# 0xC0000054/pdn-jpegxl

Hardware: AMD Instinct MI355X
Metric: megapixels/sec decode (4K lossy VarDCT) (higher is better)
Workload: dtype f32

## Files before the change

### pdn_jpegxl_amd/api.py

```python
import ctypes as C
import os

import numpy as np

from . import build as _build

DECODER_STATUS = ["Ok", "NullParameter", "InvalidParameter", "OutOfMemory", "HasAnimation", "HasMultipleFrames",
                  "ImageDimensionExceedsInt32", "UnsupportedChannelFormat", "CreateLayerError", "CreateMetadataError",
                  "DecodeError", "MetadataError", "InvalidFileSignature"]
ENCODER_STATUS = ["Ok", "NullParameter", "OutOfMemory", "UserCanceled", "EncodeError", "WriteError"]
IMAGE_FORMAT = ["Gray", "Rgb", "Cmyk"]
KNOWN_PROFILE = ["Srgb", "LinearSrgb", "LinearGray", "GraySrgbTRC", "DisplayP3", "Rec709", "Rec2020Linear", "Rec2020PQ"]
S_OK, E_ABORT, E_OUTOFMEMORY, E_FAIL = 0, -2147467260, -2147024882, -2147467259


class ErrorInfo(C.Structure):
    _fields_ = [("errorMessage", C.c_char * 256)]


class BitmapData(C.Structure):
    _fields_ = [("scan0", C.c_void_p), ("width", C.c_uint32), ("height", C.c_uint32), ("stride", C.c_uint32)]


class EncoderOptions(C.Structure):
# ... 248 lines not shown
    L = lib()
    L.jxlhip_parse_metadata.restype = C.c_size_t
    L.jxlhip_parse_metadata.argtypes = [C.c_char_p, C.c_size_t, C.c_int32, C.c_void_p, C.c_size_t, C.POINTER(C.c_int32), C.POINTER(ErrorInfo)]
    err = ErrorInfo()
    st = C.c_int32(0)
    n = L.jxlhip_parse_metadata(data, len(data), which, None, 0, C.byref(st), C.byref(err))
    if st.value != 0 or n == 0:
        return DECODER_STATUS[st.value], None, err.errorMessage.decode("ascii", "replace")
    buf = (C.c_uint8 * n)()
    L.jxlhip_parse_metadata(data, len(data), which, buf, n, C.byref(st), C.byref(err))
    return DECODER_STATUS[st.value], bytes(buf), ""


def static_table(name, index, dtype):
    L = lib()
    n = L.jxlhip_static_table(name.encode(), index, None, 0)
    buf = np.empty(n // np.dtype(dtype).itemsize, dtype)
    L.jxlhip_static_table(name.encode(), index, buf.ctypes.data, n)
    return buf


_PLANE_DTYPES = {"lf": np.float32, "lf_quant": np.int32, "cellinfo": np.uint32, "raw_quant": np.uint16, "sharpness": np.uint8,
                 "ytox": np.int8, "ytob": np.int8, "alpha": np.uint8, "inv_sigma": np.float32, "qcoef": np.int32,
                 "xyb_idct": np.float32, "xyb_filtered": np.float32}


def _last_stage_times(fn_name):
    L = lib()
    fn = getattr(L, fn_name)
    fn.restype = C.c_int32
    fn.argtypes = [C.POINTER(C.c_char_p), C.POINTER(C.c_float), C.c_int32]
    names = (C.c_char_p * 32)()
    ms = (C.c_float * 32)()
    k = fn(names, ms, 32)
    return {names[i].decode(): ms[i] for i in range(k)}


def last_load_stage_times():
    return _last_stage_times("jxlhip_last_load_stage_times")


def last_save_stage_times():
    return _last_stage_times("jxlhip_last_save_stage_times")


class Decoder:

# ... 61 lines not shown
```

### pdn_jpegxl_amd/csrc/decoder.cc

```cpp
#include <hip/hip_runtime.h>
#include <algorithm>
#include <atomic>
#include <cmath>
#include <cstdarg>
#include <cstdio>
#include <cstdlib>
#include <cstring>
#include <memory>
#include <mutex>
#include <string>
#include <thread>
#include <vector>
#include "../../include/jxlfiletypeio.h"
#include "host_parse.h"
#include "icc.h"
#include "kernels.h"

namespace jxlhip {

struct HipError : std::runtime_error {
  explicit HipError(const std::string& m) : std::runtime_error(m) {}
};
#define HIP_OK(expr)                                                                                      \
  do {                                                                                                    \
// ... 430 lines not shown
  Bump blob, ws_zero, ws;
  int n_extra = 0;
  std::vector<int> first_extra((size_t)n, 0);
  for (int i = 0; i < n; i++) {
    first_extra[i] = n + n_extra;
    if (parse_status[i] == DecoderStatus_Ok && frames[i].encoding == 0) n_extra += (int)frames[i].extra_passes.size();
  }
  const size_t off_imgs = blob.Take(sizeof(DevImage) * (size_t)(n + n_extra));
  struct PassLayout {
    size_t a_cmap, a_cfg, a_alias, a_pfx[3] = {}, lz_hf = 0, scan[kNumQuantTables] = {}, centries, cblk, bitpos, hf_order;
  };
  struct PerImg {
    std::vector<PassLayout> extra;
    size_t m_direct = 0;
    size_t sec_off, sec_size, tree, m_cmap, m_cfg, m_alias, a_cmap, a_cfg, a_alias, order[kNumOrders][3], cs;
    size_t m_pfx[3] = {}, a_pfx[3] = {};
    size_t lz_lf = 0, lz_grp = 0, lz_hf = 0, lz_mod = 0;
    size_t scan[kNumQuantTables] = {};
    size_t trc_lut = 0;
    size_t dq[kNumQuantTables] = {};
    size_t z_cellinfo, z_status, centries, cblk, hf_order;
    std::vector<size_t> mod_planes;
    size_t mod_chan, mod_desc, wp_lf, wp_grp, lf_end, alpha32;
    size_t lf[3], lf_tmp[3], lfq[3], lf_extra, rawq, sharp, ytox, ytob, binfo, lf_desc, lf_count, alpha_desc, blk_list, blk_count, bitpos, tile_list, tmp[3], xyb[3], inv_sigma, alpha;
    size_t orient_tmp = 0;
    size_t layer_px = 0;
  };
  std::vector<PerImg> L((size_t)n);
  std::vector<size_t> file_cs((size_t)S.nfiles, 0);
  std::vector<uint8_t> cs_put((size_t)S.nfiles, 0);
  auto take_cs = [&](int i) {
    const ParsedFrame& f = frames[i];
    if (!f.is_layer) return blob.Take(f.cs_size + 16);
    size_t& o = file_cs[S.file_of[i]];
    if (!o) o = blob.Take(f.cs_size + 16) + 1;
    return o - 1;
  };
  const size_t z_status_base = ws_zero.Take((size_t)std::max(1, n) * 64);
  int total_lf = 0, total_groups = 0, n_mod_tasks = 0;
  int mod_lanes = 64, mod_rb = 0, mod_wp_lds = 0;
  size_t total_mod_sections = 0;
  for (int i = 0; i < n; i++) {
    if (parse_status[i] != DecoderStatus_Ok || frames[i].encoding != 1) continue;
    if (!frames[i].tree_row_static && frames[i].group_dim <= 256) mod_rb = 256;
    if (frames[i].tree_uses_wp && frames[i].group_dim <= 256) { mod_wp_lds = 1; mod_lanes = 8; }
    total_mod_sections += frames[i].single ? 1 : 1 + (size_t)frames[i].nlf + frames[i].ng;
  }
// ... 77 lines not shown
          if (l.dq[q] || !ep.custom_order[o][0].empty() || !ep.custom_order[o][1].empty() || !ep.custom_order[o][2].empty()) pl.scan[q] = blob.Take(8 * 3 * (size_t)dq_n[q], 256) + 1;
        }
        pl.centries = ws.Take((size_t)std::max(1, g1 - g0) * f.xg * kGroupEntriesCap * 4);
        pl.cblk = ws.Take(3 * cells * sizeof(U32x2));
        pl.bitpos = ws.Take((size_t)f.ng * 8);
        pl.hf_order = blob.Take(4 * (size_t)std::max<uint32_t>(1, f.ng));
        l.extra.push_back(pl);
      }
    }
    for (int c = 0; c < 3; c++) { l.lf[c] = ws.Take(4 * cells); l.lf_tmp[c] = ws.Take(4 * cells); l.lfq[c] = ws.Take(4 * cells); }
    l.lf_extra = ws.Take(f.nlf);
    l.rawq = ws.Take(2 * cells);
    l.sharp = ws.Take(cells);
    l.ytox = ws.Take(tiles);
    l.ytob = ws.Take(tiles);
    l.binfo = ws.Take((size_t)f.nlf * kBinfoInts * 4);
    l.lf_desc = ws.Take((size_t)f.nlf * 8 * sizeof(ChanDesc));
    l.lf_count = ws.Take((size_t)f.nlf * 4);
    l.alpha_desc = ws.Take((size_t)f.ng * sizeof(ChanDesc));
    l.blk_list = ws.Take((size_t)f.ng * 1024 * 4);
    l.blk_count = ws.Take((size_t)f.ng * 4);
    l.bitpos = ws.Take((size_t)f.ng * 8);
    l.tile_list = ws.Take(tiles * 4);
    l.alpha32 = ws.Take(4 * (size_t)f.xsize * f.ysize);
    chunk_pix = std::max(chunk_pix, pix);
    l.inv_sigma = ws.Take(4 * cells);
    l.alpha = ws.Take((size_t)f.xsize * f.ysize * OutBytesPerSample(f));
    if (f.is_layer) l.layer_px = ws.Take((size_t)f.xsize * f.ysize * (f.ncolor + (f.alpha_index >= 0 ? 1 : 0)) * OutBytesPerSample(f));
    l.lf_end = ws.Take(8);
    if (f.tree_uses_wp) { l.wp_lf = ws.Take((size_t)f.nlf * kWpLfInts * 4); l.wp_grp = ws.Take((size_t)f.ng * 10 * (kGroupDim + 2) * 4); }
    {
      int b0 = 0, b1 = (int)f.yg;
      if (band_rows > 0) { b0 = std::min<int>(band_first_row, (int)f.yg); b1 = std::min<int>(b0 + band_rows, (int)f.yg); }
      const int g0 = std::max(0, b0 - 1), g1 = std::min<int>((int)f.yg, b1 + 1);
      total_lf += ((g1 + 7) / 8 - g0 / 8) * (int)f.xlf;
      total_groups += (g1 - g0) * (int)f.xg * (int)f.num_passes;
    }
  }
  const int pixel_chunk = debug_taps ? std::max(1, n) : std::min(std::max(1, n), kPixelChunk);
  std::vector<size_t> chunk_tmp((size_t)pixel_chunk * 3), chunk_xyb((size_t)pixel_chunk * 3), chunk_coef((size_t)pixel_chunk * 3);
  if (chunk_pix)
    for (int k = 0; k < pixel_chunk * 3; k++) { chunk_tmp[k] = ws.Take(4 * chunk_pix); chunk_xyb[k] = ws.Take(4 * chunk_pix); chunk_coef[k] = ws.Take(4 * chunk_pix); }
  for (int i = 0; i < n; i++)
    if (parse_status[i] == DecoderStatus_Ok && band_rows > 0 && (band_first_row < 0 || band_first_row >= (int)frames[i].yg)) {
      parse_status[i] = DecoderStatus_DecodeError;
      parse_msg[i] = "band decode: the first group row lies outside the frame";
// ... 335 lines not shown
        double a = 0;
        for (int j = 0; j < 3; j++) a += (double)plan.from_srgb[r * 3 + j] * (double)f.opsin_inv[j * 3 + k];
        d.opsin_inv[r * 3 + k] = (float)a * (255.0f / f.intensity_target);
      }
    for (int k = 0; k < 3; k++) { d.opsin_bias[k] = f.opsin_bias[k]; d.opsin_bias_cbrt[k] = std::cbrt(f.opsin_bias[k]); }
    d.cellinfo = (uint32_t*)(wz + l.z_cellinfo);
    d.status = (uint32_t*)(wz + l.z_status);
    status_off[i] = l.z_status;
    for (int c = 0; c < 3; c++) {
      d.coef[c] = (int32_t*)(wr + chunk_coef[(size_t)(i % pixel_chunk) * 3 + c]);
      d.lf[c] = (float*)(wr + l.lf[c]); d.lf_tmp[c] = (float*)(wr + l.lf_tmp[c]); d.lfq[c] = (int32_t*)(wr + l.lfq[c]);
      d.lf_final[c] = d.skip_lf_smoothing ? d.lf[c] : d.lf_tmp[c];
      d.tmp[c] = (float*)(wr + chunk_tmp[(size_t)(i % pixel_chunk) * 3 + c]); d.xyb[c] = (float*)(wr + chunk_xyb[(size_t)(i % pixel_chunk) * 3 + c]);
      d.xyb2[c] = (float*)d.coef[c];
    }
    d.lf_extra = wr + l.lf_extra;
    d.rawq = (uint16_t*)(wr + l.rawq); d.sharp = wr + l.sharp;
    d.ytox = (int8_t*)(wr + l.ytox); d.ytob = (int8_t*)(wr + l.ytob);
    d.binfo = (int32_t*)(wr + l.binfo);
    d.lf_desc = (ChanDesc*)(wr + l.lf_desc); d.lf_count = (uint32_t*)(wr + l.lf_count); d.alpha_desc = (ChanDesc*)(wr + l.alpha_desc);
    d.blk_list = (uint32_t*)(wr + l.blk_list); d.blk_count = (uint32_t*)(wr + l.blk_count);
    d.grp_bitpos = (uint64_t*)(wr + l.bitpos);
    d.tile_list = (uint32_t*)(wr + l.tile_list);
    d.alpha32 = (int32_t*)(wr + l.alpha32);
    d.centries = (uint32_t*)(wr + l.centries); d.centries_g0 = d.dec_gy0 * (int32_t)f.xg;
    d.cblk = (U32x2*)(wr + l.cblk);
    d.inv_sigma = (float*)(wr + l.inv_sigma);
    d.alpha = wr + l.alpha;
    d.lf_end_bits = (uint64_t*)(wr + l.lf_end);
    d.alpha_in_global = (d.has_alpha && f.ng == 1) ? 1 : 0;
    d.lf_start_bits = f.after_lf_global_bits;
    if (f.single) {
      d.single = 1;
      d.hf_start_bits = f.hf_start_bits;
    }
    if (f.tree_uses_wp) { d.wp_lf = (int32_t*)(wr + l.wp_lf); d.wp_grp = (int32_t*)(wr + l.wp_grp); d.wp_grp_ints = 10 * (kGroupDim + 2); }
    d.out = f.orientation == 1 ? dev_out[i] : wr + l.orient_tmp;
    if (f.is_layer) d.out = wr + l.layer_px;
    float** cur = d.xyb;
    float** other = d.xyb2;
    d.fused_gab_epf1 = (!debug_taps && f.epf_iters >= 1) ? (f.epf_iters == 1 ? 1 : 2) : 0;
    d.stream_no_gab = (d.fused_gab_epf1 && (!f.gab || f.epf_iters == 3)) ? 1 : 0;
    d.stage_on[0] = (f.gab && (!d.fused_gab_epf1 || f.epf_iters == 3)) ? 1 : 0;
    d.stage_on[1] = f.epf_iters == 3;
    d.stage_on[2] = f.epf_iters >= 1 && !d.fused_gab_epf1;
    d.stage_on[3] = f.epf_iters >= 2 && !d.fused_gab_epf1;
// ... 184 lines not shown
      if (s_lf != s_hf) HIP_OK(hipStreamWaitEvent(xs, S.lf_done, 0));
      LaunchInterference(kind, wgs, lds_kb, ms, xbuf, xbytes, xs);
    }
  }
#endif
  Mark("hf_start", s_hf, 1);
  if (!(skip_stages & 2))
  LaunchHfDecode(d_imgs, (const SectionTask*)(d_blob + off_pass_tasks), npass_t, hf_waves * 64, lane_stride, hf_ring, lds_hf <= kLdsMax ? lds_hf : 0, lds_hf_lanes, s_hf);
  Mark("hf_decode", s_hf, 1);
  if (any_alpha && !(skip_stages & 4))
    LaunchAlphaAns(d_imgs, (const SectionTask*)(d_blob + off_alpha_tasks), nalpha_t, alpha_stride, lds_alpha <= kLdsMax ? lds_alpha : 0, direct_alpha, lean_mod, s_hf);
  Mark("alpha_ans", s_hf, 1);
  if (debug_taps) {
    taps.assign(n, Tap());
    LaunchExpandCoefficients(d_imgs, n, true, max_tiles, stream);
    HIP_OK(hipStreamSynchronize(stream));
    CopyPlaneTap(0);
  }
  const bool finish_on_hf = s_hf == stream || debug_taps || !Knob("JXLHIP_ALPHA_FINISH_ON_PIX");
  if (finish_on_hf) {
    if (any_alpha && !(skip_stages & 4)) LaunchAlphaFinish(d_imgs, n, max_groups, s_hf);
    Mark("alpha_finish", s_hf, 1);
  }
  if (s_hf != stream) {
    HIP_OK(hipEventRecord(S.hf_done, s_hf));
    HIP_OK(hipStreamWaitEvent(stream, S.hf_done, 0));
  }
  Mark("main_start", stream, 2);
  if (!finish_on_hf) {
    if (any_alpha && !(skip_stages & 4)) LaunchAlphaFinish(d_imgs, n, max_groups, stream);
    Mark("alpha_finish", stream, 2);
  }
  hipStream_t s_pix = (Knob("JXLHIP_PIX_ON_HF") && s_hf != stream) ? s_hf : stream;
  for (int c0 = 0; c0 < n; c0 += pixel_chunk) {
    const int cnt = std::min(pixel_chunk, n - c0);
    if (!(skip_stages & 8))
    LaunchReconTiles(d_imgs + c0, cnt, max_tiles, d_basis_all, d_basis_small, d_llf_scale, d_basis_mfma, s_pix);
    Mark("reconstruct", s_pix, 2);
    LaunchExpandCoefficients(d_imgs + c0, cnt, false, max_tiles, s_pix);
    LaunchGenericReconstruct(d_imgs + c0, cnt, d_basis_all, d_basis_small, d_llf_scale, s_pix);
    Mark("reconstruct_generic", s_pix, 2);
    if (debug_taps) { HIP_OK(hipStreamSynchronize(s_pix)); CopyPlaneTap(1); }
    if (!(skip_stages & 16))
    LaunchFilterTiles(d_imgs + c0, cnt, max_w, max_h, stage_mask, any_unfiltered, any_fused, any_fused2, s_pix);
    Mark("filters+output", s_pix, 2);
  }
// ... 289 lines not shown
}

size_t jxlhip_read_plane(JxlHipDecoder* dec, int32_t index, const char* name, int32_t channel, void* dst, size_t capacity) {
  if (!dec || !name) return 0;
  JxlHipDecoder::Slot& S = dec->Last();
  if (index < 0 || index >= S.n || S.pending) return 0;
  if (S.parse_status[index] != DecoderStatus_Ok) return 0;
  const DevImage& d = S.imgs[index];
  std::string nm(name);
  const size_t cells = (size_t)d.w8 * d.h8, pix = (size_t)d.wp * d.hp;
  const void* src = nullptr;
  size_t bytes = 0;
  bool host = false;
  const int c = std::min(2, std::max(0, channel));
  if (nm == "lf") { src = d.lf_final[c]; bytes = cells * 4; }
  else if (nm == "lf_quant") { src = d.lfq[c]; bytes = cells * 4; }
  else if (nm == "cellinfo") { src = d.cellinfo; bytes = cells * 4; }
  else if (nm == "raw_quant") { src = d.rawq; bytes = cells * 2; }
  else if (nm == "sharpness") { src = d.sharp; bytes = cells; }
  else if (nm == "ytox") { src = d.ytox; bytes = (size_t)d.wt * d.ht; }
  else if (nm == "ytob") { src = d.ytob; bytes = (size_t)d.wt * d.ht; }
  else if (nm == "alpha") { src = d.alpha; bytes = (size_t)d.w * d.h; }
  else if (nm == "inv_sigma") { src = d.inv_sigma; bytes = cells * 4; }
  else if (dec->debug_taps && (size_t)index < S.taps.size()) {
    host = true;
    if (nm == "qcoef") { src = S.taps[index].qcoef[c].data(); bytes = S.taps[index].qcoef[c].size(); }
    else if (nm == "xyb_idct") { src = S.taps[index].xyb_idct[c].data(); bytes = S.taps[index].xyb_idct[c].size(); }
    else if (nm == "xyb_filtered") { src = S.taps[index].xyb_filtered[c].data(); bytes = S.taps[index].xyb_filtered[c].size(); }
  }
  (void)pix;
  if (!src || !bytes) return 0;
  if (dst && capacity) {
    size_t nb = std::min(bytes, capacity);
    if (host) memcpy(dst, src, nb);
    else if (hipMemcpy(dst, src, nb, hipMemcpyDeviceToHost) != hipSuccess) return 0;
  }
  return bytes;
}

int32_t jxlhip_stage_times(JxlHipDecoder* dec, const char** names, float* ms, int32_t capacity) {
  if (!dec) return 0;
  JxlHipDecoder::Slot& S = dec->Last();
  int32_t k = 0;
  for (size_t i = 1; i < S.stage_names.size() && i < S.stage_ms.size() && k < capacity; i++) {
    if (S.stage_ms[i] < 0.f) continue;
    if (names) names[k] = S.stage_names[i].c_str();
// ... 211 lines not shown
```

### pdn_jpegxl_amd/csrc/dev_types.h

```cpp
#pragma once
#include <stdint.h>

namespace jxlhip {

constexpr int kNumStrategies = 27;
constexpr int kNumOrders = 13;
constexpr int kNumQuantTables = 17;
constexpr int kGroupDim = 256;
constexpr int kGroupBlocks = 32;
constexpr int kLfGroupBlocks = 256;
constexpr int kMaxClustersLds = 128;
constexpr uint32_t kGroupEntriesCap = 3u * 65536u;

enum DevError : uint32_t {
  kErrNone = 0,
  kErrBitstream = 1u << 0,
  kErrUnsupportedHeader = 1u << 1,
  kErrUnsupportedTree = 1u << 2,
  kErrBlockLayout = 1u << 3,
  kErrRange = 1u << 4,
  kErrUnsupportedTransform = 1u << 5,
};

struct alignas(8) U32x2 { uint32_t x, y; };

struct DevTreeNode {
  int32_t property;
  int32_t splitval;
  uint32_t a;
  uint32_t b;
};

struct DevCode {
  const uint8_t* ctx_map;
  const uint32_t* cfg;
// ... 110 lines not shown
  uint32_t* lz_lf;
  uint32_t* lz_grp;
  uint32_t* lz_hf;
  uint32_t* lz_mod;
  int32_t* alpha32;
  uint32_t* centries;
  int32_t centries_g0, pad2;
  U32x2* cblk;
  int32_t* coef[3];
  float* tmp[3];
  float* xyb[3];
  float* xyb2[3];
  float* inv_sigma;
  float* stage_in[5][3];
  float* stage_out[5][3];
  int32_t stage_on[5];
  int32_t final_stage;
  int32_t fused_gab_epf1;
  float* stream_in[3];
  float* stream_mid[3];
  int32_t stream_no_gab;
  int32_t stream_pairs;
  uint32_t* tile_list;
  uint8_t* alpha;
  uint8_t* out;
  uint32_t* status;
};

struct ComposeFrame {
  const float* px;
  int32_t x0, y0, w, h;
  int32_t mode[2];
  int32_t source[2];
  int32_t clamp[2];
  int32_t save;
  int32_t pad;
};
struct ComposeImage {
  int32_t w, h, nch, has_alpha;
  int32_t premul, orientation, out_bits, out_float;
  int32_t first, count;
  int32_t raw, pad0;
  uint8_t* out;
};

constexpr int kUniGridCells = 2048;
// ... 13 lines not shown
```

### pdn_jpegxl_amd/csrc/kernels.h

```cpp
#pragma once
#include <hip/hip_runtime.h>
#include "dev_types.h"

namespace jxlhip {

void LaunchLfAns(const DevImage* imgs, const SectionTask* tasks, int ntasks, int slots, size_t lds_bytes, int scalar_rows, bool lean, hipStream_t s);
void LaunchLfFinish(const DevImage* imgs, const SectionTask* tasks, int ntasks, hipStream_t s);
void LaunchHfBlockList(const DevImage* imgs, int nimg, int max_groups, hipStream_t s);
size_t HfLaneLdsBytes(int ring_words);
void LaunchHfDecode(const DevImage* imgs, const SectionTask* tasks, int nwg, int threads, int lane_stride, int ring_words, size_t lds_bytes,
                    size_t lane_bytes, hipStream_t s);
void LaunchAlphaAns(const DevImage* imgs, const SectionTask* tasks, int nwg, int lane_stride, size_t lds_bytes, int scalar_rows, bool lean, hipStream_t s);
void LaunchAlphaFinish(const DevImage* imgs, int nimg, int max_groups, hipStream_t s);
void LaunchModularAns(const DevImage* imgs, int nimg, const SectionTask* tasks, int ntasks, size_t lds_bytes, int max_sections, int max_coded,
                      int lanes, int rb_width, int wp_lds, int scalar_rows, hipStream_t s);
void LaunchModularOp(int kind, int32_t* a, int32_t* b, int32_t* c, int aw, int ah, int rw, int rh, int type, hipStream_t s);
void LaunchModularPalette(const int32_t* palette, const int32_t* index, int32_t* const* out, int nout, int nb_colors, int w, int h, uint32_t* status,
                          hipStream_t s);
void LaunchModularOut(const DevImage* imgs, int nimg, size_t max_pixels, hipStream_t s);
void LaunchOrient(const uint8_t* src, uint8_t* dst, int w, int h, int px_bytes, int orientation, hipStream_t s);
void LaunchLfPixelStages(const DevImage* imgs, int nimg, size_t max_cells, hipStream_t s);
void LaunchExpandCoefficients(const DevImage* imgs, int nimg, bool all_tiles, int max_tiles, hipStream_t s);
void LaunchGenericReconstruct(const DevImage* imgs, int nimg, const float* basis_all, const float* basis_small,
                              const float* llf_scale, hipStream_t s);
void LaunchReconTiles(const DevImage* imgs, int nimg, int max_tiles, const float* basis_all, const float* basis_small,
                      const float* llf_scale, const float* basis_mfma, hipStream_t s);
void LaunchFilterTiles(const DevImage* imgs, int nimg, int max_w, int max_h, int stage_mask, bool any_unfiltered,
                       int any_fused, int any_fused2, hipStream_t s);

void LaunchCompose(const ComposeImage* imgs, const ComposeFrame* frames, int nimg, int max_segments, hipStream_t s);

void LaunchStatusToHost(const uint32_t* src, uint32_t* dst_pinned, int nwords, hipStream_t s);
#ifdef JXLHIP_EXPERIMENTS
void LaunchInterference(int kind, int wg_per_cu, int lds_kb, float ms, float* scratch, size_t scratch_bytes, hipStream_t s);
#endif

}
```

### pdn_jpegxl_amd/csrc/tile_kernels.hip

```cpp
#include <hip/hip_runtime.h>
#include <cstdlib>
#include "dev_types.h"
#include "dev_util.h"
#include "kernels.h"

namespace jxlhip {

#ifndef JXLHIP_PRIO_PIXEL
#define JXLHIP_PRIO_PIXEL 0
#endif
#if JXLHIP_PRIO_PIXEL
#define JXL_PIXEL_PRIO() __builtin_amdgcn_s_setprio(JXLHIP_PRIO_PIXEL)
#else
#define JXL_PIXEL_PRIO() ((void)0)
#endif

namespace {

constexpr int kTS = 64;
constexpr int kLP = 65;

__device__ const uint8_t t_quant_table[kNumStrategies] = {0, 1, 2, 3, 4, 5, 6, 6, 7, 7, 8, 8, 9, 9, 10, 10, 10, 10, 11, 12, 12, 13, 14, 14, 15, 16, 16};

__device__ __forceinline__ bool Special(uint32_t s) { return (s >= 1 && s <= 3) || (s >= 12 && s <= 17); }
// ... 135 lines not shown
}

#define JXL_IDCT_STEP(Bp, v0, v1)                                                                  \
  {                                                                                                \
    const float4 b0 = *(const float4*)(Bp);                                                        \
    const float4 b1 = *(const float4*)((Bp) + 4);                                                  \
    a0[0] += v0 * b0.x; a0[1] += v0 * b0.y; a0[2] += v0 * b0.z; a0[3] += v0 * b0.w;                \
    a0[4] += v0 * b1.x; a0[5] += v0 * b1.y; a0[6] += v0 * b1.z; a0[7] += v0 * b1.w;                \
    a1[0] += v1 * b0.x; a1[1] += v1 * b0.y; a1[2] += v1 * b0.z; a1[3] += v1 * b0.w;                \
    a1[4] += v1 * b1.x; a1[5] += v1 * b1.y; a1[6] += v1 * b1.z; a1[7] += v1 * b1.w;                \
  }

__device__ __forceinline__ float DequantBias(int32_t v, float qb, float qb3) {
  if (v == 0) return 0.f;
  if (v == 1) return qb;
  if (v == -1) return -qb;
  const float f = (float)v;
  return f - qb3 * __builtin_amdgcn_rcpf(f);
}
typedef int __attribute__((ext_vector_type(4))) I4v;

constexpr int kTileF = kTS * kLP;

__global__ __launch_bounds__(768, 6) void recon_tile_kernel(const DevImage* __restrict__ imgs, const float* basis_all, const float* basis_small,
                                                             const float* llf_scale, const float* basis_mfma) {
  JXL_PIXEL_PRIO();
  extern __shared__ __align__(16) uint8_t smem_raw[];
  float* cfc3 = (float*)smem_raw;
  float* B816 = cfc3 + 3 * kTileF;
  float* cscale = B816 + 320;
  uint32_t* ci = (uint32_t*)(cscale + 64);
  uint32_t* cmeta = ci + 64;
  uint32_t* cnq = cmeta + 64;
  uint32_t* cpre = cnq + 64;
  uint32_t* cstart = cpre + 3 * 64;
  uint32_t* ctot = cstart + 3 * 64;
  const U32x2** csc = (const U32x2**)(ctot + 4);
  float4* t32_lo = (float4*)(csc + 64);
  float4* t32_hi = t32_lo + 128;
  float4* t64 = t32_hi + 128;
  const DevImage& im = imgs[blockIdx.y];
  const int tile = blockIdx.x;
  if (tile >= im.wt * im.ht) return;
  const int tid = threadIdx.x;
  const int tx = tile % im.wt, ty = tile / im.wt;
  if (ty < im.dec_gy0 * 4 || ty >= im.dec_gy1 * 4) return;
  const int wave = tid >> 6, lane = tid & 63, team = wave >> 2, tw = wave & 3;
  const int c = team == 0 ? 1 : (team == 1 ? 0 : 2);
  const int wp = im.wp, hp = im.hp;
  {
    float4* z = (float4*)cfc3;
    for (int i = tid; i < 3 * kTileF / 4; i += 768) z[i] = make_float4(0.f, 0.f, 0.f, 0.f);
  }
  int bad = 0, has64 = 0;
  if (tid < 64) {
    const int cx = tx * 8 + (tid & 7), cy = ty * 8 + (tid >> 3);
    const bool inside = cx < im.w8 && cy < im.h8;
    const size_t cell_g = (size_t)min(cy, im.h8 - 1) * im.w8 + min(cx, im.w8 - 1);
    const size_t ncells = (size_t)im.w8 * im.h8;
    const uint32_t info_g = im.cellinfo[cell_g];
    const uint32_t rq_g = im.rawq[cell_g];
    U32x2 blk[3];
    blk[0] = im.cblk[ncells + cell_g]; blk[1] = im.cblk[cell_g]; blk[2] = im.cblk[2 * ncells + cell_g];
    const uint32_t info = inside ? info_g : 0u;
    const uint32_t rqv = inside ? rq_g : 1u;
    const int ix = (info >> 8) & 31, iy = (info >> 13) & 31, lcx = (info >> 18) & 7, lcy = (info >> 21) & 7;
    if (inside) {
      if (!(info >> 31)) bad = 1;
      else {
        const int ox = (tid & 7) - ix, oy = (tid >> 3) - iy;
        bad = ox < 0 || oy < 0 || ox + (1 << lcx) > 8 || oy + (1 << lcy) > 8 || Special(info & 0xFF) ||
              (ox & ((1 << lcx) - 1)) != 0 || (oy & ((1 << lcy) - 1)) != 0;
      }
    }
    const bool valid = (info >> 31) && !bad;
    has64 = valid && (lcx == 3 || lcy == 3);
    {
      const uint64_t any = __ballot(has64);
      if (tid == 0) ctot[3] = any != 0;
    }
    const uint32_t q = t_quant_table[valid ? (info & 0xFF) : 0];
    const uint32_t rq_origin = (uint32_t)__shfl((int)rqv, valid ? tid - iy * 8 - ix : tid);
    const uint32_t lng = 3 + max(lcx, lcy);
    const bool transposed = lcy >= lcx;
    ci[tid] = info;
    cscale[tid] = im.inv_global_scale / (float)rq_origin;
    cmeta[tid] = lng | (transposed ? 16u : 0u);
    cnq[tid] = im.dq_n[q];
    csc[tid] = im.scan[q];
    const bool origin = valid && ix == 0 && iy == 0;
    uint32_t cnt[3], sum[3];
#pragma unroll
    for (int t = 0; t < 3; t++) {
      cnt[t] = origin ? blk[t].y : 0u;
      if (cnt[t] > 65536u || blk[t].x > kGroupEntriesCap - cnt[t]) cnt[t] = 0;
      sum[t] = cnt[t];
    }
#pragma unroll
    for (int d = 1; d < 64; d <<= 1) {
#pragma unroll
      for (int t = 0; t < 3; t++) {
        const uint32_t a = (uint32_t)__shfl_up((int)sum[t], d);
        if (tid >= d) sum[t] += a;
      }
    }
#pragma unroll
    for (int t = 0; t < 3; t++) {
      cpre[t * 64 + tid] = sum[t] - cnt[t];
      cstart[t * 64 + tid] = blk[t].x;
      if (tid == 63) ctot[t] = sum[t];
    }
  } else if (tid < 64 + 320) {
    B816[tid - 64] = basis_all[tid - 64];
  } else if (tid < 64 + 320 + 256) {
    const int i = tid - (64 + 320);
    const float4 v = ((const float4*)basis_mfma)[i];
    if (i & 1) t32_hi[i >> 1] = v; else t32_lo[i >> 1] = v;
  }
  if (im.num_passes > 1) bad = 1;
  if (__syncthreads_or(bad)) {
    if (tid == 0) im.tile_list[atomicAdd(&im.status[1], 1u)] = (uint32_t)tile;
    return;
  }
  if (ctot[3]) {
    for (int i = tid; i < 1024; i += 768) t64[(i & 3) * 256 + (i >> 2)] = ((const float4*)(basis_mfma + 1024))[i];
  }
  const float* const Bl = basis_all;
  float* const cfc = cfc3 + team * kTileF;
  if (tw == 0) {
    const int cxg = tx * 8 + (lane & 7), cyg = ty * 8 + (lane >> 3);
    const bool inside = cxg < im.w8 && cyg < im.h8;
    const float lf_g = im.lf_final[c][(size_t)min(cyg, im.h8 - 1) * im.w8 + min(cxg, im.w8 - 1)];
    const float lfv = inside ? lf_g : 0.f;
    const uint32_t info = ci[lane];
    const bool valid = info >> 31;
    const int ix = (info >> 8) & 31, iy = (info >> 13) & 31, lcx = (info >> 18) & 7, lcy = (info >> 21) & 7;
    const int cx = 1 << lcx, cy = 1 << lcy;
    const int ox = (lane & 7) - ix, oy = (lane >> 3) - iy;
    const float* Bx = basis_small + (cx * cx - 1) / 3 + ix * cx;
    const float* By = basis_small + (cy * cy - 1) / 3 + iy * cy;
    float bx[8], byv[8];
#pragma unroll
    for (int k = 0; k < 8; k++) { bx[k] = (valid && k < cx) ? Bx[k] : 0.f; byv[k] = (valid && k < cy) ? By[k] : 0.f; }
    const float sc = valid ? llf_scale[lcy * 32 + iy] * llf_scale[lcx * 32 + ix] / (float)(cx * cy) : 0.f;
    float row = 0.f;
#pragma unroll
    for (int k = 0; k < 8; k++) {
      const float v = __shfl(lfv, (lane - ix + k) & 63);
      if (valid && k < cx) row += v * bx[k];
    }
    float acc = 0.f;
#pragma unroll
    for (int k = 0; k < 8; k++) {
      const float v = __shfl(row, ((oy + k) * 8 + (lane & 7)) & 63);
      if (valid && k < cy) acc += v * byv[k];
    }
    if (valid) atomicAdd(&cfc[(oy * 8 + iy) * kLP + ox * 8 + ix], acc * sc);
  }
  {
    const size_t tile_cfl = (size_t)ty * im.wt + tx;
    const float cfl_x = im.base_x + (float)im.ytox[tile_cfl] * im.inv_color_factor;
    const float cfl_b = im.base_b + (float)im.ytob[tile_cfl] * im.inv_color_factor;
    const uint32_t* entries = im.centries + (size_t)((ty >> 2) * im.xg + (tx >> 2) - im.centries_g0) * kGroupEntriesCap;
    const uint32_t t0 = ctot[0], t01 = t0 + ctot[1], total = t01 + ctot[2];
    const float qb3 = im.qbias[3];
    for (uint32_t e = (uint32_t)tid; e < total; e += 768) {
      const uint32_t t = (e >= t0) + (e >= t01);
      const uint32_t el = e - (t == 0 ? 0u : (t == 1 ? t0 : t01));
      const uint32_t* pre = cpre + t * 64;
      uint32_t j = 0;
#pragma unroll
      for (int step = 32; step; step >>= 1) if (pre[j + step] <= el) j += step;
      const uint32_t ent = entries[cstart[t * 64 + j] + (el - pre[j])];
      const uint32_t k = ent & 0xFFFFu, nq = cnq[j];
      if (k >= nq) continue;
      const int chan = t == 0 ? 1 : (t == 1 ? 0 : 2);
      const U32x2 se = csc[j][(size_t)chan * nq + k];
      const uint32_t meta = cmeta[j];
      const uint32_t lng = meta & 15, p = se.x;
      const uint32_t r = p >> lng, cc = p & ((1u << lng) - 1);
      const uint32_t ky = (meta & 16) ? cc : r, kx = (meta & 16) ? r : cc;
      if (ky >= 64 || kx >= 64) continue;
      const int32_t v = (int32_t)ent >> 16;
      const float dm = t == 0 ? 1.0f : (t == 1 ? im.x_dm : im.b_dm);
      const float o = DequantBias(v, im.qbias[chan], qb3) * (cscale[j] * dm) * __uint_as_float(se.y);
      const uint32_t at = ((j >> 3) * 8 + ky) * kLP + (j & 7) * 8 + kx;
      atomicAdd(&cfc3[t * kTileF + at], o);
      if (t == 0) {
        if (cfl_x != 0.f) atomicAdd(&cfc3[kTileF + at], o * cfl_x);
        if (cfl_b != 0.f) atomicAdd(&cfc3[2 * kTileF + at], o * cfl_b);
      }
    }
  }
  __syncthreads();
  const int l16 = tid & 15, lq = lane >> 4;
  {
    F4 acc[4];
    bool m[4];
    const int x0 = tw * 16;
#pragma unroll
    for (int rb = 0; rb < 4; rb++) {
// ... 752 lines not shown
    for (int c = 0; c < 3; c++) {
      const F2 f = (cur.c[c] + wu * prev.c[c] + wl * lft[c] + wr * rgt[c] + wd * next.c[c]) * iw;
      o[c] = skip ? cur.c[c] : f;
    }
    if (k.stores) {
      StorePixelPair(k, PixelToRgba8(im, o[0].x, o[1].x, o[2].x, al & 0xFF), PixelToRgba8(im, o[0].y, o[1].y, o[2].y, (al >> 8) & 0xFF), y - k.band_y0);
    }
    prev = cur; cur = next; next = next2; aux = aux2;
  }
}

__global__ void out_only_kernel(const DevImage* __restrict__ imgs) {
  const DevImage& im = imgs[blockIdx.y];
  if (im.final_stage != 4) return;
  const int w = im.w, wp = im.wp;
  const size_t n = (size_t)w * (im.band_y1 - im.band_y0);
  for (size_t i = (size_t)blockIdx.x * blockDim.x + threadIdx.x; i < n; i += (size_t)gridDim.x * blockDim.x) {
    const int x = (int)(i % w), y = im.band_y0 + (int)(i / w);
    const size_t o = (size_t)y * wp + x;
    WritePixel(im, x, y, im.stage_in[4][0][o], im.stage_in[4][1][o], im.stage_in[4][2][o]);
  }
}

void LaunchReconTiles(const DevImage* imgs, int nimg, int max_tiles, const float* basis_all, const float* basis_small,
                      const float* llf_scale, const float* basis_mfma, hipStream_t s) {
  const size_t lds = (size_t)(3 * kTileF + 320 + 64 * 4 + 64 * 6 + 4 + 128 + 1024 + 4096) * 4;
  static bool raised = false;
  if (!raised) { (void)hipFuncSetAttribute((const void*)recon_tile_kernel, hipFuncAttributeMaxDynamicSharedMemorySize, (int)lds); raised = true; }
  hipLaunchKernelGGL(recon_tile_kernel, dim3(max_tiles, nimg), dim3(768), lds, s, imgs, basis_all, basis_small, llf_scale, basis_mfma);
}

void LaunchFilterTiles(const DevImage* imgs, int nimg, int max_w, int max_h, int stage_mask, bool any_unfiltered,
                       int any_fused, int any_fused2, hipStream_t s) {
  const int tiles = ((max_w + 63) / 64) * ((max_h + 31) / 32);
  dim3 g(tiles, nimg);
  if (stage_mask & 1) hipLaunchKernelGGL(filter_tile_kernel<0>, g, dim3(256), 0, s, imgs);
  if (stage_mask & 2) hipLaunchKernelGGL(filter_tile_kernel<1>, g, dim3(256), 0, s, imgs);
  if (any_fused) {
    const int groups = ((max_w + kStripOut - 1) / kStripOut) * ((max_h + 2 + kSegRows - 1) / kSegRows);
    const int pair_groups = ((max_w + kPairOut - 1) / kPairOut) * ((max_h + 2 + kSegRows - 1) / kSegRows);
    if (any_fused & 1) hipLaunchKernelGGL(filter_stream_pairs_kernel, dim3((pair_groups + kGroupsPerWg - 1) / kGroupsPerWg, nimg), dim3(256), 0, s, imgs);
    if (any_fused & 2) hipLaunchKernelGGL(filter_stream_kernel, dim3((groups + kGroupsPerWg - 1) / kGroupsPerWg, nimg), dim3(256), 0, s, imgs);
    const int pair2_groups = ((max_w + kPair2Out - 1) / kPair2Out) * ((max_h + kSegRows - 1) / kSegRows);
    if (any_fused2 & 1) hipLaunchKernelGGL(filter_stream2_pairs_kernel, dim3((pair2_groups + kGroupsPerWg - 1) / kGroupsPerWg, nimg), dim3(256), 0, s, imgs);
    if (any_fused2 & 2) hipLaunchKernelGGL(filter_stream2_kernel, dim3((groups + kGroupsPerWg - 1) / kGroupsPerWg, nimg), dim3(256), 0, s, imgs);
  }
  if (stage_mask & 4) hipLaunchKernelGGL(filter_tile_kernel<2>, g, dim3(256), 0, s, imgs);
  if (stage_mask & 8) hipLaunchKernelGGL(filter_tile_kernel<3>, g, dim3(256), 0, s, imgs);
  if (any_unfiltered) {
// ... 8 lines not shown
```

Measured before the change: 30080.

## Precompute per-tile reconstruction metadata in a separate setup kernel on HF stream

Moves the per-tile cell-info validation, scale computation, prefix scans of coefficient counts and generic-tile detection out of recon_tile_kernel into a new recon_setup_kernel that writes a per-tile record to global memory. The setup kernel runs on the HF stream after alpha finish, and the recon kernel then just bulk-loads the record into LDS. It also stores precomputed per-cell entry offsets, which removes a subtraction per coefficient, and indexes the quant-table scan pointers by table id instead of per cell. In exchange it adds an extra kernel launch plus global write and read traffic for the record buffer.

```diff
diff --git a/pdn_jpegxl_amd/api.py b/pdn_jpegxl_amd/api.py
--- a/pdn_jpegxl_amd/api.py
+++ b/pdn_jpegxl_amd/api.py
@@ -294,7 +294,8 @@
 
 _PLANE_DTYPES = {"lf": np.float32, "lf_quant": np.int32, "cellinfo": np.uint32, "raw_quant": np.uint16, "sharpness": np.uint8,
                  "ytox": np.int8, "ytob": np.int8, "alpha": np.uint8, "inv_sigma": np.float32, "qcoef": np.int32,
-                 "xyb_idct": np.float32, "xyb_filtered": np.float32}
+                 "xyb_idct": np.float32, "xyb_filtered": np.float32,
+                 "cblk": np.uint32, "tile_rec": np.uint32}
 
 
 def _last_stage_times(fn_name):
diff --git a/pdn_jpegxl_amd/csrc/decoder.cc b/pdn_jpegxl_amd/csrc/decoder.cc
--- a/pdn_jpegxl_amd/csrc/decoder.cc
+++ b/pdn_jpegxl_amd/csrc/decoder.cc
@@ -476,7 +476,7 @@
     size_t z_cellinfo, z_status, centries, cblk, hf_order;
     std::vector<size_t> mod_planes;
     size_t mod_chan, mod_desc, wp_lf, wp_grp, lf_end, alpha32;
-    size_t lf[3], lf_tmp[3], lfq[3], lf_extra, rawq, sharp, ytox, ytob, binfo, lf_desc, lf_count, alpha_desc, blk_list, blk_count, bitpos, tile_list, tmp[3], xyb[3], inv_sigma, alpha;
+    size_t lf[3], lf_tmp[3], lfq[3], lf_extra, rawq, sharp, ytox, ytob, binfo, lf_desc, lf_count, alpha_desc, blk_list, blk_count, bitpos, tile_list, tile_rec, tmp[3], xyb[3], inv_sigma, alpha;
     size_t orient_tmp = 0;
     size_t layer_px = 0;
   };
@@ -600,6 +600,7 @@
     l.blk_count = ws.Take((size_t)f.ng * 4);
     l.bitpos = ws.Take((size_t)f.ng * 8);
     l.tile_list = ws.Take(tiles * 4);
+    l.tile_rec = ws.Take(tiles * kRecWords * 4);
     l.alpha32 = ws.Take(4 * (size_t)f.xsize * f.ysize);
     chunk_pix = std::max(chunk_pix, pix);
     l.inv_sigma = ws.Take(4 * cells);
@@ -981,6 +982,7 @@
     d.blk_list = (uint32_t*)(wr + l.blk_list); d.blk_count = (uint32_t*)(wr + l.blk_count);
     d.grp_bitpos = (uint64_t*)(wr + l.bitpos);
     d.tile_list = (uint32_t*)(wr + l.tile_list);
+    d.tile_rec = (uint32_t*)(wr + l.tile_rec);
     d.alpha32 = (int32_t*)(wr + l.alpha32);
     d.centries = (uint32_t*)(wr + l.centries); d.centries_g0 = d.dec_gy0 * (int32_t)f.xg;
     d.cblk = (U32x2*)(wr + l.cblk);
@@ -1211,6 +1213,8 @@
     if (any_alpha && !(skip_stages & 4)) LaunchAlphaFinish(d_imgs, n, max_groups, s_hf);
     Mark("alpha_finish", s_hf, 1);
   }
+  if (!(skip_stages & 8)) LaunchReconSetup(d_imgs, n, max_tiles, s_hf);
+  Mark("recon_setup", s_hf, 1);
   if (s_hf != stream) {
     HIP_OK(hipEventRecord(S.hf_done, s_hf));
     HIP_OK(hipStreamWaitEvent(stream, S.hf_done, 0));
@@ -1546,6 +1550,8 @@
   else if (nm == "ytob") { src = d.ytob; bytes = (size_t)d.wt * d.ht; }
   else if (nm == "alpha") { src = d.alpha; bytes = (size_t)d.w * d.h; }
   else if (nm == "inv_sigma") { src = d.inv_sigma; bytes = cells * 4; }
+  else if (nm == "cblk") { src = d.cblk; bytes = cells * 3 * sizeof(U32x2); }
+  else if (nm == "tile_rec") { src = d.tile_rec; bytes = (size_t)d.wt * d.ht * kRecWords * 4; }
   else if (dec->debug_taps && (size_t)index < S.taps.size()) {
     host = true;
     if (nm == "qcoef") { src = S.taps[index].qcoef[c].data(); bytes = S.taps[index].qcoef[c].size(); }
diff --git a/pdn_jpegxl_amd/csrc/dev_types.h b/pdn_jpegxl_amd/csrc/dev_types.h
--- a/pdn_jpegxl_amd/csrc/dev_types.h
+++ b/pdn_jpegxl_amd/csrc/dev_types.h
@@ -11,6 +11,7 @@
 constexpr int kLfGroupBlocks = 256;
 constexpr int kMaxClustersLds = 128;
 constexpr uint32_t kGroupEntriesCap = 3u * 65536u;
+constexpr int kRecCi = 0, kRecScale = 64, kRecMeta = 128, kRecPre = 192, kRecOff = 384, kRecTot = 576, kRecWords = 584;
 
 enum DevError : uint32_t {
   kErrNone = 0,
@@ -167,6 +168,7 @@
   int32_t stream_no_gab;
   int32_t stream_pairs;
   uint32_t* tile_list;
+  uint32_t* tile_rec;
   uint8_t* alpha;
   uint8_t* out;
   uint32_t* status;
diff --git a/pdn_jpegxl_amd/csrc/kernels.h b/pdn_jpegxl_amd/csrc/kernels.h
--- a/pdn_jpegxl_amd/csrc/kernels.h
+++ b/pdn_jpegxl_amd/csrc/kernels.h
@@ -23,6 +23,7 @@
 void LaunchExpandCoefficients(const DevImage* imgs, int nimg, bool all_tiles, int max_tiles, hipStream_t s);
 void LaunchGenericReconstruct(const DevImage* imgs, int nimg, const float* basis_all, const float* basis_small,
                               const float* llf_scale, hipStream_t s);
+void LaunchReconSetup(const DevImage* imgs, int nimg, int max_tiles, hipStream_t s);
 void LaunchReconTiles(const DevImage* imgs, int nimg, int max_tiles, const float* basis_all, const float* basis_small,
                       const float* llf_scale, const float* basis_mfma, hipStream_t s);
 void LaunchFilterTiles(const DevImage* imgs, int nimg, int max_w, int max_h, int stage_mask, bool any_unfiltered,
diff --git a/pdn_jpegxl_amd/csrc/tile_kernels.hip b/pdn_jpegxl_amd/csrc/tile_kernels.hip
--- a/pdn_jpegxl_amd/csrc/tile_kernels.hip
+++ b/pdn_jpegxl_amd/csrc/tile_kernels.hip
@@ -181,21 +181,89 @@
 
 constexpr int kTileF = kTS * kLP;
 
+__global__ __launch_bounds__(256) void recon_setup_kernel(const DevImage* __restrict__ imgs) {
+  const DevImage& im = imgs[blockIdx.y];
+  const int tile = blockIdx.x * 4 + (threadIdx.x >> 6);
+  if (tile >= im.wt * im.ht) return;
+  const int tx = tile % im.wt, ty = tile / im.wt;
+  if (ty < im.dec_gy0 * 4 || ty >= im.dec_gy1 * 4) return;
+  const int lane = threadIdx.x & 63;
+  uint32_t* rec = im.tile_rec + (size_t)tile * kRecWords;
+  const int cx = tx * 8 + (lane & 7), cy = ty * 8 + (lane >> 3);
+  const bool inside = cx < im.w8 && cy < im.h8;
+  const size_t cell_g = (size_t)min(cy, im.h8 - 1) * im.w8 + min(cx, im.w8 - 1);
+  const size_t ncells = (size_t)im.w8 * im.h8;
+  const uint32_t info_g = im.cellinfo[cell_g];
+  const uint32_t rq_g = im.rawq[cell_g];
+  U32x2 blk[3];
+  blk[0] = im.cblk[ncells + cell_g]; blk[1] = im.cblk[cell_g]; blk[2] = im.cblk[2 * ncells + cell_g];
+  const uint32_t info = inside ? info_g : 0u;
+  const uint32_t rqv = inside ? rq_g : 1u;
+  const int ix = (info >> 8) & 31, iy = (info >> 13) & 31, lcx = (info >> 18) & 7, lcy = (info >> 21) & 7;
+  int bad = 0;
+  if (inside) {
+    if (!(info >> 31)) bad = 1;
+    else {
+      const int ox = (lane & 7) - ix, oy = (lane >> 3) - iy;
+      bad = ox < 0 || oy < 0 || ox + (1 << lcx) > 8 || oy + (1 << lcy) > 8 || Special(info & 0xFF) ||
+            (ox & ((1 << lcx) - 1)) != 0 || (oy & ((1 << lcy) - 1)) != 0;
+    }
+  }
+  const bool valid = (info >> 31) && !bad;
+  const bool has64 = valid && (lcx == 3 || lcy == 3);
+  const uint32_t q = t_quant_table[valid ? (info & 0xFF) : 0];
+  const uint32_t rq_origin = (uint32_t)__shfl((int)rqv, valid ? lane - iy * 8 - ix : lane);
+  const uint32_t lng = 3 + max(lcx, lcy);
+  const bool transposed = lcy >= lcx;
+  rec[kRecCi + lane] = info;
+  rec[kRecScale + lane] = __float_as_uint(im.inv_global_scale / (float)rq_origin);
+  rec[kRecMeta + lane] = lng | (transposed ? 16u : 0u) | (q << 8);
+  const bool origin = valid && ix == 0 && iy == 0;
+  uint32_t cnt[3], sum[3];
+#pragma unroll
+  for (int t = 0; t < 3; t++) {
+    cnt[t] = origin ? blk[t].y : 0u;
+    if (cnt[t] > 65536u || blk[t].x > kGroupEntriesCap - cnt[t]) cnt[t] = 0;
+    sum[t] = cnt[t];
+  }
+#pragma unroll
+  for (int d = 1; d < 64; d <<= 1) {
+#pragma unroll
+    for (int t = 0; t < 3; t++) {
+      const uint32_t a = (uint32_t)__shfl_up((int)sum[t], d);
+      if (lane >= d) sum[t] += a;
+    }
+  }
+#pragma unroll
+  for (int t = 0; t < 3; t++) {
+    rec[kRecPre + t * 64 + lane] = sum[t] - cnt[t];
+    rec[kRecOff + t * 64 + lane] = blk[t].x - (sum[t] - cnt[t]);
+    if (lane == 63) rec[kRecTot + t] = sum[t];
+  }
+  const bool to_generic = __ballot(bad) != 0 || im.num_passes > 1;
+  const bool any64 = __ballot(has64) != 0;
+  if (lane == 0) {
+    rec[kRecTot + 3] = (any64 ? 1u : 0u) | (to_generic ? 2u : 0u);
+    if (to_generic) im.tile_list[atomicAdd(&im.status[1], 1u)] = (uint32_t)tile;
+  }
+}
+
 __global__ __launch_bounds__(768, 6) void recon_tile_kernel(const DevImage* __restrict__ imgs, const float* basis_all, const float* basis_small,
                                                              const float* llf_scale, const float* basis_mfma) {
   JXL_PIXEL_PRIO();
   extern __shared__ __align__(16) uint8_t smem_raw[];
   float* cfc3 = (float*)smem_raw;
   float* B816 = cfc3 + 3 * kTileF;
-  float* cscale = B816 + 320;
-  uint32_t* ci = (uint32_t*)(cscale + 64);
-  uint32_t* cmeta = ci + 64;
-  uint32_t* cnq = cmeta + 64;
-  uint32_t* cpre = cnq + 64;
-  uint32_t* cstart = cpre + 3 * 64;
-  uint32_t* ctot = cstart + 3 * 64;
-  const U32x2** csc = (const U32x2**)(ctot + 4);
-  float4* t32_lo = (float4*)(csc + 64);
+  uint4* smem_rec = (uint4*)(B816 + 320);
+  uint32_t* ci = (uint32_t*)smem_rec + kRecCi;
+  float* cscale = (float*)smem_rec + kRecScale;
+  uint32_t* cmeta = (uint32_t*)smem_rec + kRecMeta;
+  uint32_t* cpre = (uint32_t*)smem_rec + kRecPre;
+  uint32_t* coff = (uint32_t*)smem_rec + kRecOff;
+  uint32_t* ctot = (uint32_t*)smem_rec + kRecTot;
+  uint32_t* cnq = (uint32_t*)smem_rec + kRecWords;
+  const U32x2** csc = (const U32x2**)(cnq + 32);
+  float4* t32_lo = (float4*)(csc + 32);
   float4* t32_hi = t32_lo + 128;
   float4* t64 = t32_hi + 128;
   const DevImage& im = imgs[blockIdx.y];
@@ -211,86 +279,36 @@
     float4* z = (float4*)cfc3;
     for (int i = tid; i < 3 * kTileF / 4; i += 768) z[i] = make_float4(0.f, 0.f, 0.f, 0.f);
   }
-  int bad = 0, has64 = 0;
-  if (tid < 64) {
-    const int cx = tx * 8 + (tid & 7), cy = ty * 8 + (tid >> 3);
-    const bool inside = cx < im.w8 && cy < im.h8;
-    const size_t cell_g = (size_t)min(cy, im.h8 - 1) * im.w8 + min(cx, im.w8 - 1);
-    const size_t ncells = (size_t)im.w8 * im.h8;
-    const uint32_t info_g = im.cellinfo[cell_g];
-    const uint32_t rq_g = im.rawq[cell_g];
-    U32x2 blk[3];
-    blk[0] = im.cblk[ncells + cell_g]; blk[1] = im.cblk[cell_g]; blk[2] = im.cblk[2 * ncells + cell_g];
-    const uint32_t info = inside ? info_g : 0u;
-    const uint32_t rqv = inside ? rq_g : 1u;
-    const int ix = (info >> 8) & 31, iy = (info >> 13) & 31, lcx = (info >> 18) & 7, lcy = (info >> 21) & 7;
-    if (inside) {
-      if (!(info >> 31)) bad = 1;
-      else {
-        const int ox = (tid & 7) - ix, oy = (tid >> 3) - iy;
-        bad = ox < 0 || oy < 0 || ox + (1 << lcx) > 8 || oy + (1 << lcy) > 8 || Special(info & 0xFF) ||
-              (ox & ((1 << lcx) - 1)) != 0 || (oy & ((1 << lcy) - 1)) != 0;
-      }
-    }
-    const bool valid = (info >> 31) && !bad;
-    has64 = valid && (lcx == 3 || lcy == 3);
-    {
-      const uint64_t any = __ballot(has64);
-      if (tid == 0) ctot[3] = any != 0;
-    }
-    const uint32_t q = t_quant_table[valid ? (info & 0xFF) : 0];
-    const uint32_t rq_origin = (uint32_t)__shfl((int)rqv, valid ? tid - iy * 8 - ix : tid);
-    const uint32_t lng = 3 + max(lcx, lcy);
-    const bool transposed = lcy >= lcx;
-    ci[tid] = info;
-    cscale[tid] = im.inv_global_scale / (float)rq_origin;
-    cmeta[tid] = lng | (transposed ? 16u : 0u);
-    cnq[tid] = im.dq_n[q];
-    csc[tid] = im.scan[q];
-    const bool origin = valid && ix == 0 && iy == 0;
-    uint32_t cnt[3], sum[3];
-#pragma unroll
-    for (int t = 0; t < 3; t++) {
-      cnt[t] = origin ? blk[t].y : 0u;
-      if (cnt[t] > 65536u || blk[t].x > kGroupEntriesCap - cnt[t]) cnt[t] = 0;
-      sum[t] = cnt[t];
-    }
-#pragma unroll
-    for (int d = 1; d < 64; d <<= 1) {
-#pragma unroll
-      for (int t = 0; t < 3; t++) {
-        const uint32_t a = (uint32_t)__shfl_up((int)sum[t], d);
-        if (tid >= d) sum[t] += a;
-      }
-    }
-#pragma unroll
-    for (int t = 0; t < 3; t++) {
-      cpre[t * 64 + tid] = sum[t] - cnt[t];
-      cstart[t * 64 + tid] = blk[t].x;
-      if (tid == 63) ctot[t] = sum[t];
-    }
-  } else if (tid < 64 + 320) {
-    B816[tid - 64] = basis_all[tid - 64];
-  } else if (tid < 64 + 320 + 256) {
-    const int i = tid - (64 + 320);
+  if (tid < kRecWords / 4) {
+    smem_rec[tid] = ((const uint4*)(im.tile_rec + (size_t)tile * kRecWords))[tid];
+  } else if (tid >= 160 && tid < 160 + kNumQuantTables) {
+    cnq[tid - 160] = im.dq_n[tid - 160];
+    csc[tid - 160] = im.scan[tid - 160];
+  } else if (tid >= 192 && tid < 192 + 320) {
+    B816[tid - 192] = basis_all[tid - 192];
+  } else if (tid >= 512) {
+    const int i = tid - 512;
     const float4 v = ((const float4*)basis_mfma)[i];
     if (i & 1) t32_hi[i >> 1] = v; else t32_lo[i >> 1] = v;
   }
-  if (im.num_passes > 1) bad = 1;
-  if (__syncthreads_or(bad)) {
-    if (tid == 0) im.tile_list[atomicAdd(&im.status[1], 1u)] = (uint32_t)tile;
-    return;
-  }
-  if (ctot[3]) {
-    for (int i = tid; i < 1024; i += 768) t64[(i & 3) * 256 + (i >> 2)] = ((const float4*)(basis_mfma + 1024))[i];
-  }
-  const float* const Bl = basis_all;
-  float* const cfc = cfc3 + team * kTileF;
+  float lfv = 0.f;
   if (tw == 0) {
     const int cxg = tx * 8 + (lane & 7), cyg = ty * 8 + (lane >> 3);
     const bool inside = cxg < im.w8 && cyg < im.h8;
     const float lf_g = im.lf_final[c][(size_t)min(cyg, im.h8 - 1) * im.w8 + min(cxg, im.w8 - 1)];
-    const float lfv = inside ? lf_g : 0.f;
+    lfv = inside ? lf_g : 0.f;
+  }
+  const size_t tile_cfl = (size_t)ty * im.wt + tx;
+  const float cfl_x = im.base_x + (float)im.ytox[tile_cfl] * im.inv_color_factor;
+  const float cfl_b = im.base_b + (float)im.ytob[tile_cfl] * im.inv_color_factor;
+  __syncthreads();
+  if (ctot[3] & 2u) return;
+  if (ctot[3] & 1u) {
+    for (int i = tid; i < 1024; i += 768) t64[(i & 3) * 256 + (i >> 2)] = ((const float4*)(basis_mfma + 1024))[i];
+  }
+  const float* const Bl = basis_all;
+  float* const cfc = cfc3 + team * kTileF;
+  if (tw == 0) {
     const uint32_t info = ci[lane];
     const bool valid = info >> 31;
     const int ix = (info >> 8) & 31, iy = (info >> 13) & 31, lcx = (info >> 18) & 7, lcy = (info >> 21) & 7;
@@ -317,9 +335,6 @@
     if (valid) atomicAdd(&cfc[(oy * 8 + iy) * kLP + ox * 8 + ix], acc * sc);
   }
   {
-    const size_t tile_cfl = (size_t)ty * im.wt + tx;
-    const float cfl_x = im.base_x + (float)im.ytox[tile_cfl] * im.inv_color_factor;
-    const float cfl_b = im.base_b + (float)im.ytob[tile_cfl] * im.inv_color_factor;
     const uint32_t* entries = im.centries + (size_t)((ty >> 2) * im.xg + (tx >> 2) - im.centries_g0) * kGroupEntriesCap;
     const uint32_t t0 = ctot[0], t01 = t0 + ctot[1], total = t01 + ctot[2];
     const float qb3 = im.qbias[3];
@@ -330,12 +345,12 @@
       uint32_t j = 0;
 #pragma unroll
       for (int step = 32; step; step >>= 1) if (pre[j + step] <= el) j += step;
-      const uint32_t ent = entries[cstart[t * 64 + j] + (el - pre[j])];
-      const uint32_t k = ent & 0xFFFFu, nq = cnq[j];
+      const uint32_t ent = entries[coff[t * 64 + j] + el];
+      const uint32_t meta = cmeta[j], qt = meta >> 8;
+      const uint32_t k = ent & 0xFFFFu, nq = cnq[qt];
       if (k >= nq) continue;
       const int chan = t == 0 ? 1 : (t == 1 ? 0 : 2);
-      const U32x2 se = csc[j][(size_t)chan * nq + k];
-      const uint32_t meta = cmeta[j];
+      const U32x2 se = csc[qt][(size_t)chan * nq + k];
       const uint32_t lng = meta & 15, p = se.x;
       const uint32_t r = p >> lng, cc = p & ((1u << lng) - 1);
       const uint32_t ky = (meta & 16) ? cc : r, kx = (meta & 16) ? r : cc;
@@ -1134,9 +1149,13 @@
   }
 }
 
+void LaunchReconSetup(const DevImage* imgs, int nimg, int max_tiles, hipStream_t s) {
+  hipLaunchKernelGGL(recon_setup_kernel, dim3((max_tiles + 3) / 4, nimg), dim3(256), 0, s, imgs);
+}
+
 void LaunchReconTiles(const DevImage* imgs, int nimg, int max_tiles, const float* basis_all, const float* basis_small,
                       const float* llf_scale, const float* basis_mfma, hipStream_t s) {
-  const size_t lds = (size_t)(3 * kTileF + 320 + 64 * 4 + 64 * 6 + 4 + 128 + 1024 + 4096) * 4;
+  const size_t lds = (size_t)(3 * kTileF + 320 + kRecWords + 32 + 64 + 1024 + 4096) * 4;
   static bool raised = false;
   if (!raised) { (void)hipFuncSetAttribute((const void*)recon_tile_kernel, hipFuncAttributeMaxDynamicSharedMemorySize, (int)lds); raised = true; }
   hipLaunchKernelGGL(recon_tile_kernel, dim3(max_tiles, nimg), dim3(768), lds, s, imgs, basis_all, basis_small, llf_scale, basis_mfma);
```

Result: no change. 30330, median of 6 (+0.8%).
